# mattmireles/Mamba-ASR

Hardware: AMD Instinct MI355X
Metric: encoder audio-frames/sec (ConMamba-large, L=4000) (higher is better)
Workload: dtype bf16; 1 GPU; conmamba_large_ctc: encoder forward, 64 utterances x 4000 frames (1000 scan steps) per GPU, random-init weights; global_batch=64, frames_per_utterance=4000, parallelism=utterance shards x1 (no collective in forward), launch=hipGraph replay, streams=2 (join)

## Files before the change

### mamba_asr_amd/csrc/cnn_front.hip

```cpp
#include "cm_common.h"

namespace {

typedef __attribute__((ext_vector_type(8))) __bf16 bf16x8;
typedef __attribute__((ext_vector_type(2))) __bf16 bf16x2;
typedef __attribute__((ext_vector_type(4))) float f32x4;
typedef __attribute__((ext_vector_type(2))) float f32x2;

constexpr int F0 = 80;
constexpr int C1 = 64, F1 = 40, F1P = 42;
constexpr int C2 = 32, F2 = 20;
constexpr int TT = 4;
constexpr int NR = 2 * TT + 1;
constexpr int CS = 68;
constexpr int OTS = 36;
constexpr int FW = 84;
constexpr int NB = (TT * F2 + 15) / 16;

__device__ __forceinline__ int reflect_idx(int i, int n) { return i < 0 ? -i : (i >= n ? 2 * n - 2 - i : i); }
__device__ __forceinline__ float wave_sum64(float v) {
    v = cm_group_sum<16>(v);
    v += __shfl_xor(v, 16, 64);
    v += __shfl_xor(v, 32, 64);
    return v;
}
__device__ __forceinline__ uint32_t pack2(float a, float b) {
    return __builtin_bit_cast(uint32_t, __builtin_convertvector(f32x2{a, b}, bf16x2));
}

struct front_lds {
    uint16_t rows[NR][F1P][CS];
    float ot[NB * 16][OTS];
    float fin[8][3][2][FW];
    float ln1[2][F1 * C1];
    bf16x8 wfrag[2][18][64];
};

__global__ __launch_bounds__(512) void cnn_front_kernel(const cm_cnn_front_args p, int T1, int T2, int tiles_per_utt, int chunk, int chunks_per_utt,
                                                        int nchunks) {
    extern __shared__ __attribute__((aligned(16))) unsigned char smem[];
    front_lds &L = *reinterpret_cast<front_lds *>(smem);
    const int tid = threadIdx.x, lane = tid & 63;
    const int wave = __builtin_amdgcn_readfirstlane(tid >> 6);
    const int l15 = lane & 15, lq = lane >> 4;
    const int T = p.T, T1P = T1 + 2;

    const uint16_t *W2 = reinterpret_cast<const uint16_t *>(p.w2);
    for (int i = tid; i < 2 * 18 * 64; i += 512) {
        const int cb = i / (18 * 64), ks = (i / 64) % 18, ln = i % 64;
        L.wfrag[cb][ks][ln] = *reinterpret_cast<const bf16x8 *>(W2 + ((int64_t)(cb * 16 + (ln & 15)) * 9 + (ks >> 1)) * C1 + (ks & 1) * 32 + (ln >> 4) * 8);
    }
    float4 bias2[2];
#pragma unroll
    for (int cb = 0; cb < 2; ++cb)
        bias2[cb] = p.b2 ? *reinterpret_cast<const float4 *>(p.b2 + cb * 16 + lq * 4) : make_float4(0.f, 0.f, 0.f, 0.f);
    const int cp = lane & 31, fh = lane >> 5;
    f32x2 w1[9];
#pragma unroll
    for (int k = 0; k < 9; ++k) w1[k] = f32x2{p.w1[(2 * cp) * 9 + k], p.w1[(2 * cp + 1) * 9 + k]};
    const float b1a = p.b1 ? p.b1[2 * cp] : 0.f, b1b = p.b1 ? p.b1[2 * cp + 1] : 0.f;
    for (int i = tid; i < F1 * C1; i += 512) { L.ln1[0][i] = p.ln1_g[i]; L.ln1[1][i] = p.ln1_b[i]; }

    const int pidx = min(wave * 16 + l15, TT * F2 - 1);
    const int pr = pidx / F2, pf = pidx % F2;
    uint16_t *out = reinterpret_cast<uint16_t *>(p.out);

    auto fetch_rows = [&](const float *feats, int tp, float (&r)[4]) {
        const int t1 = reflect_idx(min(tp, T1P - 1) - 1, T1);
#pragma unroll
        for (int k = 0; k < 4; ++k) {
            const int idx = lane + 64 * k;
            r[k] = 0.f;
            if (idx < 3 * 82) {
                const int rr = idx / 82, fc = idx - rr * 82;
                r[k] = feats[(int64_t)reflect_idx(2 * t1 + rr - 1, T) * F0 + reflect_idx(fc - 1, F0)];
            }
        }
    };
    auto stage_rows = [&](const float (&r)[4]) {
#pragma unroll
        for (int k = 0; k < 4; ++k) {
            const int idx = lane + 64 * k;
            if (idx < 3 * 82) {
                const int rr = idx / 82, fc = idx % 82;
                L.fin[wave][rr][0][fc] = r[k];
                if (fc >= 2) L.fin[wave][rr][1][fc - 2] = r[k];
            }
        }
    };
    auto block1_row = [&](int slot) {
        float v[2 * (F1 / 2)];
        float s = 0.f;
#pragma unroll
        for (int i = 0; i < F1 / 2; ++i) {
            f32x2 a2 = {b1a, b1b};
#pragma unroll
            for (int dt = 0; dt < 3; ++dt) {
                const f32x4 xv = *reinterpret_cast<const f32x4 *>(&L.fin[wave][dt][fh][4 * i]);
#pragma unroll
                for (int df = 0; df < 3; ++df) a2 = __builtin_elementwise_fma(w1[dt * 3 + df], f32x2{xv[df], xv[df]}, a2);
            }
            v[2 * i] = a2.x; v[2 * i + 1] = a2.y;
            s += a2.x + a2.y;
            if (i & 1) __builtin_amdgcn_sched_barrier(0);
        }
        const float mean = wave_sum64(s) * (1.f / (F1 * C1));
        float sq = 0.f;
#pragma unroll
        for (int i = 0; i < F1; ++i) { v[i] -= mean; sq = fmaf(v[i], v[i], sq); }
        const float rstd = rsqrtf(wave_sum64(sq) * (1.f / (F1 * C1)) + p.eps1);
#pragma unroll
        for (int i = 0; i < F1 / 2; ++i) {
            const int f1 = 2 * i + fh, o = f1 * C1 + 2 * cp;
            const float2 g = *reinterpret_cast<const float2 *>(&L.ln1[0][o]);
            const float2 bt = *reinterpret_cast<const float2 *>(&L.ln1[1][o]);
            float y0 = fmaf(v[2 * i] * rstd, g.x, bt.x), y1 = fmaf(v[2 * i + 1] * rstd, g.y, bt.y);
            y0 = y0 > 0.f ? y0 : p.slope * y0;
            y1 = y1 > 0.f ? y1 : p.slope * y1;
            const uint32_t pk = pack2(y0, y1);
            *reinterpret_cast<uint32_t *>(&L.rows[slot][f1 + 1][2 * cp]) = pk;
            if (f1 == 1) *reinterpret_cast<uint32_t *>(&L.rows[slot][0][2 * cp]) = pk;
            if (f1 == F1 - 2) *reinterpret_cast<uint32_t *>(&L.rows[slot][F1P - 1][2 * cp]) = pk;
        }
    };

    for (int ch = blockIdx.x; ch < nchunks; ch += gridDim.x) {
        const int b = ch / chunks_per_utt, tile0 = (ch % chunks_per_utt) * chunk;
        const int tile1 = min(tile0 + chunk, tiles_per_utt);
        const float *feats = p.feats + (int64_t)b * T * F0;
        float pre[4];
        __syncthreads();
        if (wave == 0) {
            fetch_rows(feats, 2 * TT * tile0, pre);
            stage_rows(pre);
            block1_row((2 * TT * tile0) % NR);
        }
        fetch_rows(feats, 2 * TT * tile0 + 1 + wave, pre);
        for (int tile = tile0; tile < tile1; ++tile) {
            const int tp0 = 2 * TT * tile, r0 = TT * tile;
            stage_rows(pre);
            if (tile + 1 < tile1) fetch_rows(feats, tp0 + 2 * TT + 1 + wave, pre);
            block1_row((tp0 + 1 + wave) % NR);
            cm_lds_barrier();
            if (wave < NB) {
                f32x4 acc0 = {0.f, 0.f, 0.f, 0.f}, acc1 = {0.f, 0.f, 0.f, 0.f};
                const uint16_t *fr[3];
#pragma unroll
                for (int dt = 0; dt < 3; ++dt) fr[dt] = &L.rows[(tp0 + 2 * pr + dt) % NR][2 * pf][lq * 8];
#pragma unroll
                for (int ks = 0; ks < 18; ++ks) {
                    const int tap = ks >> 1, dt = tap / 3, df = tap % 3;
                    const bf16x8 bfr = *reinterpret_cast<const bf16x8 *>(fr[dt] + df * CS + (ks & 1) * 32);
                    acc0 = __builtin_amdgcn_mfma_f32_16x16x32_bf16(L.wfrag[0][ks][lane], bfr, acc0, 0, 0, 0);
                    acc1 = __builtin_amdgcn_mfma_f32_16x16x32_bf16(L.wfrag[1][ks][lane], bfr, acc1, 0, 0, 0);
                }
                float *o = &L.ot[wave * 16 + l15][lq * 4];
                *reinterpret_cast<float4 *>(o) = make_float4(acc0[0] + bias2[0].x, acc0[1] + bias2[0].y, acc0[2] + bias2[0].z, acc0[3] + bias2[0].w);
                *reinterpret_cast<float4 *>(o + 16) = make_float4(acc1[0] + bias2[1].x, acc1[1] + bias2[1].y, acc1[2] + bias2[1].z, acc1[3] + bias2[1].w);
            }
            cm_lds_barrier();
            if (wave < TT && r0 + wave < T2) {
                constexpr int nfeat = F2 * C2;
                const float *orow = &L.ot[wave * F2][0];
                float2 vv[nfeat / 128];
                float s = 0.f;
#pragma unroll
                for (int k = 0; k < nfeat / 128; ++k) {
                    const int i = lane + 64 * k;
                    vv[k] = *reinterpret_cast<const float2 *>(orow + (i >> 4) * OTS + 2 * (i & 15));
                    s += vv[k].x + vv[k].y;
                }
                const float mean = wave_sum64(s) * (1.f / nfeat);
                float sq = 0.f;
#pragma unroll
                for (int k = 0; k < nfeat / 128; ++k) {
                    vv[k].x -= mean; vv[k].y -= mean;
                    sq = fmaf(vv[k].x, vv[k].x, fmaf(vv[k].y, vv[k].y, sq));
                }
                const float rstd = rsqrtf(wave_sum64(sq) * (1.f / nfeat) + p.eps2);
                uint16_t *dst = out + ((int64_t)b * T2 + r0 + wave) * nfeat;
#pragma unroll
                for (int k = 0; k < nfeat / 128; ++k) {
                    const int i = lane + 64 * k;
                    const float2 g = *reinterpret_cast<const float2 *>(p.ln2_g + 2 * i);
                    const float2 bt = *reinterpret_cast<const float2 *>(p.ln2_b + 2 * i);
                    float y0 = fmaf(vv[k].x * rstd, g.x, bt.x), y1 = fmaf(vv[k].y * rstd, g.y, bt.y);
                    y0 = y0 > 0.f ? y0 : y0 * p.slope;
                    y1 = y1 > 0.f ? y1 : y1 * p.slope;
                    *reinterpret_cast<uint32_t *>(dst + 2 * i) = pack2(y0, y1);
                }
            }
            cm_lds_barrier();
        }
    }
}

}

extern "C" int cm_cnn_front(const cm_cnn_front_args *args) {
    CM_REQUIRE(args != nullptr, CM_EINVAL, "cnn_front: args is NULL");
    const cm_cnn_front_args &a = *args;
    CM_REQUIRE(a.batch > 0 && a.T >= 5 && a.feats && a.w1 && a.ln1_g && a.ln1_b && a.w2 && a.ln2_g && a.ln2_b && a.out, CM_EINVAL,
               "cnn_front: bad sizes or NULL tensor");
    CM_REQUIRE(a.F == F0 && a.C1 == C1 && a.C2 == C2, CM_EUNSUPPORTED, "cnn_front: only 80 bins, channels (64, 32) (got F %d, C %d, %d)", a.F,
               a.C1, a.C2);
    CM_REQUIRE(cm_aligned(a.w2, 16) && cm_aligned(a.out, 4) && cm_aligned(a.ln1_g, 8) && cm_aligned(a.ln1_b, 8) && cm_aligned(a.ln2_g, 8) &&
                   cm_aligned(a.ln2_b, 8) && (!a.b2 || cm_aligned(a.b2, 16)),
               CM_EALIGN, "cnn_front: w2 / b2 must be 16-byte aligned, LayerNorm parameters 8-byte aligned");
    const int T1 = (a.T + 1) / 2, T2 = (T1 + 2 - 3) / 2 + 1;
    const int tiles_per_utt = (T2 + TT - 1) / TT;
    const int chunk = 16;
    const int chunks_per_utt = (tiles_per_utt + chunk - 1) / chunk;
    const int64_t nchunks = (int64_t)a.batch * chunks_per_utt;
    CM_REQUIRE(nchunks <= 2147483647, CM_EINVAL, "cnn_front: too many chunks");
    static bool attr_done = false;
    if (!attr_done) {
        hipError_t e = hipFuncSetAttribute(reinterpret_cast<const void *>(cnn_front_kernel), hipFuncAttributeMaxDynamicSharedMemorySize, 150 * 1024);
        if (e != hipSuccess) {
            cm_set_error("cnn_front: hipFuncSetAttribute failed: %s", hipGetErrorString(e));
            return (int)e;
        }
        attr_done = true;
    }
    const int64_t grid = nchunks < 256 ? nchunks : 256;
    hipLaunchKernelGGL(cnn_front_kernel, dim3((unsigned)grid), dim3(512), sizeof(front_lds), reinterpret_cast<hipStream_t>(a.stream), a, T1, T2,
                       tiles_per_utt, chunk, chunks_per_utt, (int)nchunks);
    return cm_launch_status("cm_cnn_front");
}
```

### mamba_asr_amd/fused.py

```python
from __future__ import annotations

import os
from typing import Dict, Optional

import torch
import torch.nn.functional as F

from . import ops, weight_cache


class _LayerCache:

    def __init__(self, layer, dtype):
        self.dtype = dtype
        c = lambda t: t.detach().to(dtype).contiguous()
        f = lambda t: None if t is None else t.detach().float().contiguous()
        ffn = lambda m: dict(ln=(f(m[0].weight), f(m[0].bias), m[0].eps), w1=c(m[1].ffn[0].weight), b1=c(m[1].ffn[0].bias),
                             w2=c(m[1].ffn[3].weight), b2=c(m[1].ffn[3].bias), b1f=f(m[1].ffn[0].bias),
                             b2f=f(m[1].ffn[3].bias))
        self.ffn1, self.ffn2 = ffn(layer.ffn_module1), ffn(layer.ffn_module2)
        if ops.ffn_supported(self.ffn1["w1"].shape[1], self.ffn1["w1"].shape[0], dtype) and self.ffn1["w1"].is_cuda:
            for q in (self.ffn1, self.ffn2):
                q["w1p"], q["w2p"] = ops.PackedWeight(q["w1"], ops.FFN_LAYOUT), ops.PackedWeight(q["w2"], ops.FFN_LAYOUT)
                if ops.SMALL_FFN_ROWS > 0:
# ... 125 lines not shown
        xz = h @ c.in_proj.t()
        if c.in_bias is not None:
            xz = xz + c.in_bias
    xz3 = xz.view(batch, seqlen, 2 * E)
    ucat = torch.empty((batch, seqlen, 2 * E), dtype=xz.dtype, device=xz.device)
    xdbl = None
    if USE_CONV_XPROJ and USE_SCAN_ROWS and c.rows_mode and c.wx_packed is not None and xz.dtype == torch.bfloat16:
        xdbl = ops.conv_xproj(xz3[:, :, :E], c.dirs[0]["conv_w"], c.dirs[0]["conv_b"], c.dirs[1]["conv_w"], c.dirs[1]["conv_b"],
                              c.wx_packed[0], c.wx_packed[1], out_f=ucat[:, :, :E], out_b=ucat[:, :, E:])
    else:
        ops.conv_cl_fwd(xz3[:, :, :E], c.dirs[0]["conv_w"], c.dirs[0]["conv_b"], c.dirs[1]["conv_w"], c.dirs[1]["conv_b"],
                        True, out_f=ucat[:, :, :E], out_b=ucat[:, :, E:])
    ycat = torch.empty_like(ucat)
    dirs = _scan_dirs(c, ucat, ycat, batch, seqlen, xdbl)
    ops.scan_cl_fwd(dirs, z=xz3[:, :, E:], delta_softplus=True)
    y = ycat.view(rows, 2 * E) @ c.out_cat.t()
    if c.out_bias is not None:
        y = y + c.out_bias
    if c.gamma is not None:
        y = y * c.gamma.to(y.dtype)
    return y


USE_FUSED_FFN = os.environ.get("CM_FUSED_FFN", "1") == "1"


USE_LN_PW_GLU = os.environ.get("CM_LN_PW_GLU", "1") == "1"


def _layer_forward_ffn_fused(c, x, batch, seqlen, dtype, final_ln=None):
    D = x.shape[-1]
    f1, f2 = c.ffn1, c.ffn2
    if 0 < x.shape[0] <= ops.SMALL_FFN_ROWS and "w1s" in f1:
        f1 = dict(f1, w1p=f1["w1s"], w2p=f1["w2s"])
        f2 = dict(f2, w1p=f2["w1s"], w2p=f2["w2s"])
        inp = getattr(c, "in_packed_s", None)
    else:
        inp = c.in_packed
    if c.in_packed is not None:
        _, xz = ops.ffn_fused(x, f1["ln"], f1["w1p"], f1["b1f"], f1["w2p"], f1["b2f"], alpha=0.5, norm2=c.norm1, proj_w=inp)
        y = bimamba_fused(c, None, batch, seqlen, xz=xz)
    else:
        _, h = ops.ffn_fused(x, f1["ln"], f1["w1p"], f1["b1f"], f1["w2p"], f1["b2f"], alpha=0.5, norm2=c.norm1)
        y = bimamba_fused(c, h, batch, seqlen)
    if USE_LN_PW_GLU and c.pw_packed is not None and y.dtype == torch.bfloat16 and y.is_contiguous():
        gl = ops.ln_pw_glu(x, y, 1.0, c.cm_ln, c.pw_packed, c.pw_bf)
        g = ops.glu_dwconv_ln_gelu(gl.view(batch, seqlen, D), c.dw_w, c.dw_b, c.cm_ln2[0], c.cm_ln2[1], c.cm_ln2[2],
                                   weight_t=c.dw_wt, glu_done=True, lin_w=c.lin_packed, lin_b=c.lin_bf)
    else:
        _, h = ops.add_layernorm(x, y, 1.0, x_out=x, norm2=c.cm_ln, out_dtype=dtype)
        pw = torch.addmm(c.pw_b, h, c.pw_w.t()).view(batch, seqlen, 2 * D)
        g = ops.glu_dwconv_ln_gelu(pw, c.dw_w, c.dw_b, c.cm_ln2[0], c.cm_ln2[1], c.cm_ln2[2], weight_t=c.dw_wt,
                                   lin_w=c.lin_packed, lin_b=c.lin_bf)
    y = g if c.lin_packed is not None else torch.addmm(c.lin_b, g.view(-1, D), c.lin_w.t())
    if final_ln is not None:
        _, out = ops.ffn_fused(x, f2["ln"], f2["w1p"], f2["b1f"], f2["w2p"], f2["b2f"], alpha=0.5, addend=y.view(-1, D),
                               norm1=c.norm2, norm2=final_ln, h_dtype=torch.float32)
        return out, None
    ops.ffn_fused(x, f2["ln"], f2["w1p"], f2["b1f"], f2["w2p"], f2["b2f"], alpha=0.5, addend=y.view(-1, D), norm1=c.norm2,
                  want_h=False)
    return x, None


def layer_forward(layer, x, batch, seqlen, dtype, next_ln=None, final_ln=None):
    c = _cache(layer, dtype)
    D = x.shape[-1]
    if USE_FUSED_FFN and ops.ffn_supported(D, c.ffn1["w1"].shape[0], dtype) and c.ffn2["w1"].shape[0] == c.ffn1["w1"].shape[0]:
        return _layer_forward_ffn_fused(c, x, batch, seqlen, dtype, final_ln)
    _, h = ops.add_layernorm(x, None, norm2=c.ffn1["ln"], out_dtype=dtype)
    y = _ffn(x, h, c.ffn1, dtype)
    _, h = ops.add_layernorm(x, y, 0.5, x_out=x, norm2=c.norm1, out_dtype=dtype)
    y = bimamba_fused(c, h, batch, seqlen)
    _, h = ops.add_layernorm(x, y, 1.0, x_out=x, norm2=c.cm_ln, out_dtype=dtype)
    pw = torch.addmm(c.pw_b, h, c.pw_w.t()).view(batch, seqlen, 2 * D)
    g = ops.glu_dwconv_ln_gelu(pw, c.dw_w, c.dw_b, c.cm_ln2[0], c.cm_ln2[1], c.cm_ln2[2], weight_t=c.dw_wt)
    y = torch.addmm(c.lin_b, g.view(-1, D), c.lin_w.t())
    _, h = ops.add_layernorm(x, y, 1.0, x_out=x, norm2=c.ffn2["ln"], out_dtype=dtype)
    y = _ffn(x, h, c.ffn2, dtype)
    n1 = c.norm2
    if final_ln is not None:
        ops.add_layernorm(x, y, 0.5, x_out=x, norm1=n1, want_out=False)
        _, out = ops.add_layernorm(x, None, norm2=final_ln, out_dtype=torch.float32)
        return out, None
    ops.add_layernorm(x, y, 0.5, x_out=x, norm1=n1, want_out=False)
    return x, None



USE_NATIVE_GEMM = os.environ.get("CM_NATIVE_GEMM", "0") == "1"


def _native_gemms_ok(c: _LayerCache, D: int, dtype) -> bool:
    F_ = c.ffn1["w1"].shape[0]
    return (USE_NATIVE_GEMM and dtype == torch.bfloat16 and D == 256 and F_ % 256 == 0 and F_ % 64 == 0 and (2 * c.d_inner) % 256 == 0
            and c.gamma is None)


def layer_forward_native(layer, x, h, batch, seqlen, next_ln):
    c = _cache(layer, torch.bfloat16)
    D, E, R, N = x.shape[-1], c.d_inner, c.dt_rank, c.d_state
    rows = batch * seqlen
    g = ops.gemm_bf16
    u1 = g(h, c.ffn1["w1"], c.ffn1["b1f"], epilogue=1)
    h = g(u1, c.ffn1["w2"], c.ffn1["b2f"], epilogue=2, x=x, alpha=0.5, norm2=c.norm1)
    xz = g(h, c.in_proj, c.in_bias_f, epilogue=0)
    xz3 = xz.view(batch, seqlen, 2 * E)
    ucat = torch.empty((batch, seqlen, 2 * E), dtype=xz.dtype, device=xz.device)
    ops.conv_cl_fwd(xz3[:, :, :E], c.dirs[0]["conv_w"], c.dirs[0]["conv_b"], c.dirs[1]["conv_w"], c.dirs[1]["conv_b"],
                    True, out_f=ucat[:, :, :E], out_b=ucat[:, :, E:])
    ycat = torch.empty_like(ucat)
    dirs = _scan_dirs(c, ucat, ycat, batch, seqlen)
    ops.scan_cl_fwd(dirs, z=xz3[:, :, E:], delta_softplus=True)
    h = g(ycat.view(rows, 2 * E), c.out_cat, c.out_bias_f, epilogue=2, x=x, alpha=1.0, norm2=c.cm_ln)
    pw = g(h, c.pw_w, c.pw_bf, epilogue=0).view(batch, seqlen, 2 * D)
    gl = ops.glu_dwconv_ln_gelu(pw, c.dw_w, c.dw_b, c.cm_ln2[0], c.cm_ln2[1], c.cm_ln2[2], weight_t=c.dw_wt)
    h = g(gl.view(rows, D), c.lin_w, c.lin_bf, epilogue=2, x=x, alpha=1.0, norm2=c.ffn2["ln"])
    u2 = g(h, c.ffn2["w1"], c.ffn2["b1f"], epilogue=1)
    return g(u2, c.ffn2["w2"], c.ffn2["b2f"], epilogue=2, x=x, alpha=0.5, norm1=c.norm2, norm2=next_ln,
             want_out=next_ln is not None)


N_STREAMS = int(os.environ.get("CM_STREAMS", "2"))
STREAM_MODE = os.environ.get("CM_STREAM_MODE", "join")
_side_streams = {}


def _encoder_forward_joined(encoder, src, dtype, ns, paired=False):
    batch, seqlen, D = src.shape
    if dtype != torch.bfloat16 or not USE_FUSED_FFN or not (USE_CONV_XPROJ and USE_SCAN_ROWS and USE_LN_PW_GLU):
        return None
    caches = [_cache(layer, dtype) for layer in encoder.layers]
    for c in caches:
        if not (ops.ffn_supported(D, c.ffn1["w1"].shape[0], dtype) and c.ffn2["w1"].shape[0] == c.ffn1["w1"].shape[0] and c.rows_mode
                and c.wx_packed is not None and c.pw_packed is not None and c.in_bias is None and c.out_bias is None and c.gamma is None):
            return None
    dev = src.device
    cur = torch.cuda.current_stream(dev)
    pool = _side_streams.setdefault(dev.index, [])
    while len(pool) < ns - 1:
        pool.append(torch.cuda.Stream(device=dev))
    streams = [cur] + pool[:ns - 1]
    edges = [int(round(i * batch / ns)) for i in range(ns + 1)]
    parts = [(edges[i], edges[i + 1]) for i in range(ns) if edges[i + 1] > edges[i]]
    E = caches[0].d_inner
    n = len(encoder.layers)
    fin = (encoder.norm.norm.weight.detach().float(), encoder.norm.norm.bias.detach().float(), encoder.norm.norm.eps)
    with torch.autocast("cuda", enabled=False):
        x = src.detach().float().reshape(batch * seqlen, D).contiguous()
        if x.data_ptr() == src.data_ptr():
            x = x.clone()
        xz = torch.empty((batch, seqlen, 2 * E), dtype=dtype, device=dev)
        ucat, ycat = torch.empty_like(xz), torch.empty_like(xz)
        xdbl = torch.empty((batch, seqlen, 96), dtype=dtype, device=dev)
        outs = [None] * len(parts)

        def fork():
            for st in streams[1:len(parts)]:
                st.wait_stream(cur)

        def join():
            for st in streams[1:len(parts)]:
                cur.wait_stream(st)

        fork()
        gate = None
        for li, c in enumerate(caches):
            f1, f2 = c.ffn1, c.ffn2
            for pi, (b0, b1) in enumerate(parts):
                with torch.cuda.stream(streams[pi]):
                    xp = x[b0 * seqlen:b1 * seqlen]
                    if c.in_packed is not None:
                        ops.ffn_fused(xp, f1["ln"], f1["w1p"], f1["b1f"], f1["w2p"], f1["b2f"], alpha=0.5, norm2=c.norm1,
                                      proj_w=c.in_packed, proj_out=xz[b0:b1].view(-1, 2 * E))
                    else:
                        _, h = ops.ffn_fused(xp, f1["ln"], f1["w1p"], f1["b1f"], f1["w2p"], f1["b2f"], alpha=0.5, norm2=c.norm1)
                        torch.mm(h, c.in_proj.t(), out=xz[b0:b1].view(-1, 2 * E))
                    ops.conv_xproj(xz[b0:b1, :, :E], c.dirs[0]["conv_w"], c.dirs[0]["conv_b"], c.dirs[1]["conv_w"], c.dirs[1]["conv_b"],
                                   c.wx_packed[0], c.wx_packed[1], out_f=ucat[b0:b1, :, :E], out_b=ucat[b0:b1, :, E:], xdbl=xdbl[b0:b1])
            if paired:
                for pi, (b0, b1) in enumerate(parts):
                    with torch.cuda.stream(streams[pi]):
                        if gate is not None:
                            streams[pi].wait_event(gate)
                        ops.scan_cl_fwd(_scan_dirs(c, ucat[b0:b1], ycat[b0:b1], b1 - b0, seqlen, xdbl[b0:b1]), z=xz[b0:b1, :, E:],
                                        delta_softplus=True)
                        gate = torch.cuda.Event()
                        gate.record(streams[pi])
            else:
                join()
                ops.scan_cl_fwd(_scan_dirs(c, ucat, ycat, batch, seqlen, xdbl), z=xz[:, :, E:], delta_softplus=True)
                fork()
            for pi, (b0, b1) in enumerate(parts):
                with torch.cuda.stream(streams[pi]):
                    xp = x[b0 * seqlen:b1 * seqlen]
                    y = ycat[b0:b1].view(-1, 2 * E) @ c.out_cat.t()
                    gl = ops.ln_pw_glu(xp, y, 1.0, c.cm_ln, c.pw_packed, c.pw_bf)
                    g = ops.glu_dwconv_ln_gelu(gl.view(b1 - b0, seqlen, D), c.dw_w, c.dw_b, c.cm_ln2[0], c.cm_ln2[1], c.cm_ln2[2],
                                               weight_t=c.dw_wt, glu_done=True, lin_w=c.lin_packed, lin_b=c.lin_bf)
                    yl = g.view(-1, D) if c.lin_packed is not None else torch.addmm(c.lin_b, g.view(-1, D), c.lin_w.t())
                    if li == n - 1:
                        _, outs[pi] = ops.ffn_fused(xp, f2["ln"], f2["w1p"], f2["b1f"], f2["w2p"], f2["b2f"], alpha=0.5, addend=yl,
                                                    norm1=c.norm2, norm2=fin, h_dtype=torch.float32)
                    else:
                        ops.ffn_fused(xp, f2["ln"], f2["w1p"], f2["b1f"], f2["w2p"], f2["b2f"], alpha=0.5, addend=yl, norm1=c.norm2,
                                      want_h=False)
        join()
        for o in outs[1:]:
            o.record_stream(cur)
        return torch.cat(outs, dim=0).view(batch, seqlen, D)


@torch.no_grad()
def encoder_forward(encoder, src, dtype: Optional[torch.dtype] = None, streams: Optional[int] = None):
    if dtype is None:
        dtype = torch.get_autocast_dtype("cuda") if torch.is_autocast_enabled("cuda") else torch.float32
    ns = min(N_STREAMS, max(1, src.shape[0] // 16)) if streams is None else streams
    if ns > 1 and src.shape[0] >= 2 * 8 and STREAM_MODE in ("join", "pair"):
        out = _encoder_forward_joined(encoder, src, dtype, ns, paired=STREAM_MODE == "pair")
        if out is not None:
            return out
    if ns > 1 and src.shape[0] >= 2 * 8:
        dev = src.device
        cur = torch.cuda.current_stream(dev)
        pool = _side_streams.setdefault(dev.index, [torch.cuda.Stream(device=dev) for _ in range(ns - 1)])
        chunks = list(torch.chunk(src, ns, dim=0))
        outs = [None] * len(chunks)
        for i in range(1, len(chunks)):
            pool[i - 1].wait_stream(cur)
            with torch.cuda.stream(pool[i - 1]):
                outs[i] = encoder_forward(encoder, chunks[i], dtype, streams=1)
        outs[0] = encoder_forward(encoder, chunks[0], dtype, streams=1)
        for i in range(1, len(chunks)):
            cur.wait_stream(pool[i - 1])
            outs[i].record_stream(cur)
        return torch.cat(outs, dim=0)
    batch, seqlen, D = src.shape
    with torch.autocast("cuda", enabled=False):
        x = src.detach().float().reshape(batch * seqlen, D).contiguous()
        if x.data_ptr() == src.data_ptr():
            x = x.clone()
        n = len(encoder.layers)
        fin = (encoder.norm.norm.weight.detach().float(), encoder.norm.norm.bias.detach().float(), encoder.norm.norm.eps)
        caches = [_cache(layer, dtype) for layer in encoder.layers]
        if all(_native_gemms_ok(c, D, dtype) for c in caches):
            _, h = ops.add_layernorm(x, None, norm2=caches[0].ffn1["ln"], out_dtype=dtype)
            for i, layer in enumerate(encoder.layers):
                h = layer_forward_native(layer, x, h, batch, seqlen, caches[i + 1].ffn1["ln"] if i + 1 < n else None)
            _, out = ops.add_layernorm(x, None, norm2=fin, out_dtype=torch.float32)
            return out.view(batch, seqlen, D)
        out = x
        for i, layer in enumerate(encoder.layers):
            out, _ = layer_forward(layer, x, batch, seqlen, dtype, final_ln=fin if i == n - 1 else None)
        return out.view(batch, seqlen, D)


USE_CNN_FRONT = os.environ.get("CM_CNN_FRONT", "1") == "1"


def _frontend_bundle(model, dtype):
    b0, b1 = model.CNN.blocks
    lin = model.Transformer.custom_src_module.layers[0].w
    return dict(w2=b1.conv.weight.detach().to(dtype).contiguous(memory_format=torch.channels_last),
                b2=b1.conv.bias.detach().to(dtype), b2f=b1.conv.bias.detach().float().contiguous(),
                w2_ohwi=b1.conv.weight.detach().to(dtype).permute(0, 2, 3, 1).contiguous(),
                ln2=(b1.norm.norm.weight.detach().float().reshape(-1).contiguous(),
                     b1.norm.norm.bias.detach().float().reshape(-1).contiguous(), b1.norm.norm.eps),
                lin_w=lin.weight.detach().to(dtype).contiguous(), lin_b=lin.bias.detach().to(dtype))


_FRONTEND = weight_cache.Kind("_cm_frontend_cache", graphs_read=False, build=_frontend_bundle)


def _frontend_cache(model, dtype):
    return _FRONTEND.lookup(model, _params_key(dtype, model.CNN, model.Transformer.custom_src_module), dtype)


@torch.no_grad()
def asr_encode(model, wavs, wav_lens, dtype: Optional[torch.dtype] = None):
    if dtype is None:
        dtype = torch.get_autocast_dtype("cuda") if torch.is_autocast_enabled("cuda") else torch.float32
    with torch.autocast("cuda", enabled=False):
        feats = model.compute_features(wavs, norm=(model.normalize.glob_mean, model.normalize.glob_std))
        c = _frontend_cache(model, dtype)
        b0 = model.CNN.blocks[0]
        if (USE_CNN_FRONT and dtype == torch.bfloat16 and ops.cnn_front_supported(feats, b0.conv.weight, c["w2_ohwi"])
                and b0.norm.norm.weight.numel() == 40 * 64):
            src = ops.cnn_front(feats, b0.conv.weight, b0.conv.bias, b0.norm.norm.weight, b0.norm.norm.bias, b0.norm.norm.eps,
                                c["w2_ohwi"], c["b2f"], c["ln2"][0], c["ln2"][1], c["ln2"][2], 0.01)
            batch, t2 = src.shape[0], src.shape[1]
            x = torch.addmm(c["lin_b"], src.view(batch * t2, -1), c["lin_w"].t())
            return encoder_forward(model.Transformer.encoder, x.view(batch, t2, -1), dtype)
        y1 = ops.cnn_block1(feats, b0.conv.weight, b0.conv.bias, b0.norm.norm.weight, b0.norm.norm.bias,
                            b0.norm.norm.eps, 0.01, out_dtype=dtype, pad_out=1)
        if dtype == torch.bfloat16 and tuple(c["w2_ohwi"].shape) == (32, 3, 3, 64):
            src = ops.cnn_block2(y1, c["w2_ohwi"], c["b2f"], c["ln2"][0], c["ln2"][1], c["ln2"][2], 0.01)
            batch, t2 = src.shape[0], src.shape[1]
            x = torch.addmm(c["lin_b"], src.view(batch * t2, -1), c["lin_w"].t())
            return encoder_forward(model.Transformer.encoder, x.view(batch, t2, -1), dtype)
        y2 = F.conv2d(y1.permute(0, 3, 1, 2), c["w2"], c["b2"], stride=2)
        y2 = y2.permute(0, 2, 3, 1)
        if not y2.is_contiguous():
            y2 = y2.contiguous()
        batch, t2 = y2.shape[0], y2.shape[1]
        _, src = ops.add_layernorm(None, y2.reshape(batch * t2, -1), norm2=c["ln2"], out_dtype=dtype, out_act=1)
        x = torch.addmm(c["lin_b"], src, c["lin_w"].t())
        return encoder_forward(model.Transformer.encoder, x.view(batch, t2, -1), dtype)


class GraphedEncode:

    def __init__(self, model, wavs, wav_lens, dtype=torch.bfloat16, warmup: int = 2):
        self.model, self.dtype = model, dtype
        self.wavs, self.lens = wavs.clone(), wav_lens.clone()
        side = torch.cuda.Stream(device=wavs.device)
        side.wait_stream(torch.cuda.current_stream(wavs.device))
        with torch.cuda.stream(side):
            for _ in range(warmup):
                self._run()
        torch.cuda.current_stream(wavs.device).wait_stream(side)
        self.graph = torch.cuda.CUDAGraph()
        with torch.cuda.graph(self.graph):
            self.out = self._run()

    def _run(self):
        with torch.no_grad(), torch.autocast("cuda", dtype=self.dtype, enabled=self.dtype != torch.float32):
            return self.model.encode(self.wavs, self.lens)

    def __call__(self, wavs=None, wav_lens=None):
        if wavs is not None:
            self.wavs.copy_(wavs)
        if wav_lens is not None:
            self.lens.copy_(wav_lens)
        self.graph.replay()
        return self.out
```

### mamba_asr_amd/ops.py

```python
from __future__ import annotations

import ctypes as ct
from typing import Optional, Tuple

import math
import os

import torch

from . import _native as N
from . import weight_cache
from .weight_cache import invalidate_caches

_DT = {torch.float32: N.CM_F32, torch.bfloat16: N.CM_BF16, torch.float16: N.CM_F16}


DETERMINISTIC = os.environ.get("CM_DETERMINISTIC", "1") == "1"


LAUNCH_LOG: Optional[list] = None


def _launch(name: str, fn, args, units: int = 0):
    log = LAUNCH_LOG
# ... 1362 lines not shown
    b, l, d2 = inp.shape
    d = d2 if glu_done else d2 // 2
    w = _f32c(weight).reshape(d, -1)
    bs, g, bt = _f32c(bias), _f32c(ln_weight), _f32c(ln_bias)
    out = torch.empty((b, l, d), dtype=inp.dtype, device=inp.device)
    a = N.GluDwconvArgs()
    a.batch, a.seqlen, a.dim, a.ksize, a.io_dtype, a.glu_done = b, l, d, w.shape[1], _DT[inp.dtype], int(bool(glu_done))
    a.in_, a.weight, a.bias, a.ln_g, a.ln_b, a.eps, a.out = _ptr(inp), _ptr(w), _ptr(bs), _ptr(g), _ptr(bt), float(eps), _ptr(out)
    wt = w.t().contiguous() if weight_t is None else weight_t
    if wt.dtype != torch.float32 or wt.shape != (w.shape[1], d) or not wt.is_contiguous():
        raise RuntimeError("glu_dwconv_ln_gelu: weight_t must be a contiguous fp32 (k, dim) tensor")
    a.weight_t = _ptr(wt)
    if lin_w is not None:
        if not isinstance(lin_w, PackedWeight) or lin_w.shape != (d, d) or lin_b is None:
            raise RuntimeError("glu_dwconv_ln_gelu: lin_w must be a PackedWeight of shape (dim, dim), with lin_b")
        lb = _f32c(lin_b)
        a.lin_w, a.lin_b = _ptr(lin_w.data), _ptr(lb)
    a.stream, a.variant = _stream(), int(variant)
    _launch("cm_glu_dwconv_ln_gelu", N.lib().cm_glu_dwconv_ln_gelu, a, units=b * l)
    return out


def cnn_block1(feats, weight, bias, ln_weight, ln_bias, eps=1e-5, slope=0.01, out_dtype=torch.bfloat16, pad_out=1):
    _dev_check(feats, weight, bias, ln_weight, ln_bias)
    feats = feats.float().contiguous()
    b, t, f = feats.shape
    w, bs, g, bt = _f32c(weight), _f32c(bias), _f32c(ln_weight), _f32c(ln_bias)
    cch = w.shape[0]
    t1, f1 = (t + 1) // 2, (f + 1) // 2
    out = torch.empty((b, t1 + 2 * pad_out, f1 + 2 * pad_out, cch), dtype=out_dtype, device=feats.device)
    a = N.CnnBlock1Args()
    a.batch, a.T, a.F, a.C, a.io_dtype, a.pad_out = b, t, f, cch, _DT[out_dtype], pad_out
    a.feats, a.weight, a.bias, a.ln_g, a.ln_b, a.eps, a.slope, a.out = (_ptr(feats), _ptr(w), _ptr(bs), _ptr(g), _ptr(bt),
                                                                          float(eps), float(slope), _ptr(out))
    a.stream = _stream()
    _launch("cm_cnn_block1", N.lib().cm_cnn_block1, a, units=b * t)
    return out


def cnn_front_supported(feats, w1, w2_ohwi) -> bool:
    return (feats.shape[-1] == 80 and tuple(w1.shape) == (64, 1, 3, 3) and tuple(w2_ohwi.shape) == (32, 3, 3, 64)
            and w2_ohwi.dtype == torch.bfloat16 and feats.shape[1] >= 5)


def cnn_front(feats, w1, b1, ln1_w, ln1_b, eps1, w2_ohwi, b2, ln2_w, ln2_b, eps2, slope=0.01):
    _dev_check(feats, w1, b1, ln1_w, ln1_b, w2_ohwi, b2, ln2_w, ln2_b)
    feats = feats.float().contiguous()
    if not cnn_front_supported(feats, w1, w2_ohwi) or not w2_ohwi.is_contiguous():
        raise RuntimeError("cnn_front: needs 80 bins, a (64, 1, 3, 3) first conv and a contiguous bf16 (32, 3, 3, 64) second conv")
    b, t, f = feats.shape
    t1 = (t + 1) // 2
    t2 = (t1 - 1) // 2 + 1
    w1f, b1f, g1, bt1 = _f32c(w1), _f32c(b1), _f32c(ln1_w).reshape(-1), _f32c(ln1_b).reshape(-1)
    b2f, g2, bt2 = _f32c(b2), _f32c(ln2_w).reshape(-1), _f32c(ln2_b).reshape(-1)
    if g1.numel() != 40 * 64 or g2.numel() != 20 * 32:
        raise RuntimeError("cnn_front: LayerNorm parameters must have 40*64 and 20*32 elements")
    out = torch.empty((b, t2, 640), dtype=torch.bfloat16, device=feats.device)
    a = N.CnnFrontArgs()
    a.batch, a.T, a.F, a.C1, a.C2 = b, t, f, 64, 32
    a.feats, a.w1, a.b1, a.ln1_g, a.ln1_b = _ptr(feats), _ptr(w1f), _ptr(b1f), _ptr(g1), _ptr(bt1)
    a.w2, a.b2, a.ln2_g, a.ln2_b = _ptr(w2_ohwi), _ptr(b2f), _ptr(g2), _ptr(bt2)
    a.eps1, a.eps2, a.slope, a.out, a.stream = float(eps1), float(eps2), float(slope), _ptr(out), _stream()
    _launch("cm_cnn_front", N.lib().cm_cnn_front, a, units=b * t)
    return out


def cnn_block2(y1, weight_ohwi, bias, ln_weight, ln_bias, eps=1e-5, slope=0.01):
    _dev_check(y1, weight_ohwi, bias, ln_weight, ln_bias)
    if y1.dtype != torch.bfloat16 or not y1.is_contiguous() or y1.dim() != 4:
        raise RuntimeError("cnn_block2: input must be a contiguous bf16 (batch, T, F, C) tensor")
    if weight_ohwi.dtype != torch.bfloat16 or not weight_ohwi.is_contiguous() or weight_ohwi.dim() != 4:
        raise RuntimeError("cnn_block2: weight must be a contiguous bf16 (C_out, 3, 3, C_in) tensor")
    b, t, f, cin = y1.shape
    cout = weight_ohwi.shape[0]
    if tuple(weight_ohwi.shape[1:]) != (3, 3, cin):
        raise RuntimeError("cnn_block2: weight shape does not match the input channels / 3x3 taps")
    t2, f2 = (t - 3) // 2 + 1, (f - 3) // 2 + 1
    bs, g, bt = _f32c(bias), _f32c(ln_weight).reshape(-1), _f32c(ln_bias).reshape(-1)
    if g.numel() != f2 * cout or bt.numel() != f2 * cout:
        raise RuntimeError("cnn_block2: LayerNorm parameters must have F2 * C_out elements")
    out = torch.empty((b, t2, f2 * cout), dtype=torch.bfloat16, device=y1.device)
    a = N.CnnBlock2Args()
    a.batch, a.T_in, a.F_in, a.C_in, a.C_out = b, t, f, cin, cout
    a.in_, a.weight, a.bias, a.ln_g, a.ln_b, a.eps, a.slope, a.out = (_ptr(y1), _ptr(weight_ohwi), _ptr(bs), _ptr(g), _ptr(bt),
                                                                      float(eps), float(slope), _ptr(out))
    a.stream = _stream()
    _launch("cm_cnn_block2", N.lib().cm_cnn_block2, a, units=b * t2)
    return out


def gemm_supported(m: int, n: int, k: int, epilogue: int) -> bool:
    return k % 64 == 0 and n % 256 == 0 and (epilogue != 2 or n == 256)


def gemm_bf16(a, w, bias=None, epilogue=0, x=None, alpha=1.0, norm1=None, norm2=None, want_out=True):
    _dev_check(a, w, bias, x)
    if a.dtype != torch.bfloat16 or w.dtype != torch.bfloat16 or a.dim() != 2 or a.stride(1) != 1 or not w.is_contiguous():
        raise RuntimeError("gemm_bf16: a must be a (M, K) bf16 row-major view and w a contiguous (N, K) bf16 tensor")
    m, k = a.shape
    n = w.shape[0]
    g = N.GemmArgs()
    g.M, g.N, g.K, g.epilogue = m, n, k, epilogue
    g.A, g.lda, g.W, g.ldw, g.bias = _ptr(a), a.stride(0), _ptr(w), w.stride(0), _ptr(bias)
    out = None
    if epilogue != 2 or want_out:
        out = torch.empty((m, n), dtype=torch.bfloat16, device=a.device)
        g.out, g.ldo = _ptr(out), n
    if epilogue == 2:
        if x is None or x.dtype != torch.float32 or not x.is_contiguous() or x.shape != (m, n):
            raise RuntimeError("gemm_bf16: epilogue 2 needs a contiguous fp32 residual x of shape (M, N)")
        g.x, g.alpha = _ptr(x), float(alpha)
        if norm1 is not None:
            g.g1, g.b1, g.eps1 = _ptr(norm1[0]), _ptr(norm1[1]), float(norm1[2])
        if norm2 is not None:
            g.g2, g.b2, g.eps2 = _ptr(norm2[0]), _ptr(norm2[1]), float(norm2[2])
    g.stream = _stream()
    _launch("cm_gemm_bf16", N.lib().cm_gemm_bf16, g, units=m)
    return out


def ffn_supported(d_model: int, hidden: int, dtype) -> bool:
    return dtype == torch.bfloat16 and d_model == 256 and hidden >= 256 and hidden % 256 == 0


FFN_LAYOUT = 32 if os.environ.get("CM_FFN_MFMA32", "0") == "1" else 16
SMALL_FFN_ROWS = int(os.environ.get("CM_FFN_SMALL_ROWS", "0"))


class PackedWeight:

    def __init__(self, w: torch.Tensor, layout: int = 16):
        _dev_check(w)
        if w.dtype != torch.bfloat16 or w.dim() != 2:
            raise RuntimeError("PackedWeight: expected a 2-D bf16 tensor")
        if layout not in (16, 32):
            raise RuntimeError("PackedWeight: layout must be 16 or 32")
        w = w.contiguous()
        self.shape = tuple(w.shape)
        self.layout = layout
        self.data = torch.empty(w.numel(), dtype=torch.bfloat16, device=w.device)
        self.repack_(w)

    def repack_(self, w: torch.Tensor) -> "PackedWeight":
        if w.dtype != torch.bfloat16 or tuple(w.shape) != self.shape or w.device != self.data.device:
            raise RuntimeError("PackedWeight.repack_: expected a bf16 tensor of the packed shape on the image's device")
        w = w.contiguous()
        fn = N.lib().cm_ffn_pack_weights if self.layout == 16 else N.lib().cm_ffn_pack_weights32
        rc = fn(_ptr(w), w.shape[0], w.shape[1], _ptr(self.data), _stream())
        N.check(rc, "cm_ffn_pack_weights")
        return self


def ffn_fused(x, pre_norm, w1, b1, w2, b2, alpha=0.5, addend=None, add_scale=1.0, norm1=None, norm2=None,
              x_out=None, want_h=True, h_dtype=torch.bfloat16, proj_w=None, proj_b=None, proj_out=None, train=None, tokens=None):
    _dev_check(x, b1, b2, addend, proj_b)
    rows, d = x.shape
    if x.dtype != torch.float32 or not x.is_contiguous():
        raise RuntimeError("ffn_fused: x must be a contiguous fp32 (rows, 256) tensor")
    if d != 256:
        raise RuntimeError(f"ffn_fused: d_model must be 256 (got {d})")
    lay = w1.layout if isinstance(w1, PackedWeight) else (w2.layout if isinstance(w2, PackedWeight) else (16 if train is not None else FFN_LAYOUT))
    w1 = w1 if isinstance(w1, PackedWeight) else PackedWeight(w1, lay)
    w2 = w2 if isinstance(w2, PackedWeight) else PackedWeight(w2, lay)
    if w1.shape[1] != d or w2.shape != (d, w1.shape[0]):
        raise RuntimeError("ffn_fused: weight shapes do not match x")
    if w1.layout != w2.layout or (proj_w is not None and isinstance(proj_w, PackedWeight) and proj_w.layout != w1.layout):
        raise RuntimeError("ffn_fused: w1, w2 and proj_w must be packed in the same layout")
    if train is not None and w1.layout != 16:
        raise RuntimeError("ffn_fused: the training forward takes layout-16 weights")
    for t in (b1, b2) + tuple(pre_norm[:2]):
        if t.dtype != torch.float32:
            raise RuntimeError("ffn_fused: biases and LayerNorm parameters must be fp32")
    a = N.FfnArgs()
    a.rows, a.dim, a.hidden = rows, d, w1.shape[0]
    a.x, a.pre_g, a.pre_b, a.pre_eps = _ptr(x), _ptr(pre_norm[0]), _ptr(pre_norm[1]), float(pre_norm[2])
    a.w1, a.b1, a.w2, a.b2, a.alpha = _ptr(w1.data), _ptr(b1), _ptr(w2.data), _ptr(b2), float(alpha)
    a.layout = 1 if w1.layout == 32 else 0
    if w1.layout == 32:
        a.tokens = int(tokens) if tokens else (32 if rows <= SMALL_FFN_ROWS else 64)
    if addend is not None:
        if addend.dtype != torch.bfloat16 or not addend.is_contiguous() or addend.shape != x.shape:
            raise RuntimeError("ffn_fused: addend must be a contiguous bf16 tensor shaped like x")
        a.addend, a.add_scale = _ptr(addend), float(add_scale)
    if norm1 is not None:
        a.n1_g, a.n1_b, a.n1_eps = _ptr(norm1[0]), _ptr(norm1[1]), float(norm1[2])
    if norm2 is not None:
        a.n2_g, a.n2_b, a.n2_eps = _ptr(norm2[0]), _ptr(norm2[1]), float(norm2[2])
    xo = x if x_out is None else x_out
    a.x_out = _ptr(xo)
    h = None
    if train is not None:
        if addend is not None or norm1 is not None or norm2 is not None or proj_w is not None:
            raise RuntimeError("ffn_fused: the training forward takes no addend / norm1 / norm2 / projection")
        pre = torch.empty((rows, w1.shape[0]), dtype=torch.bfloat16, device=x.device)
        xn = torch.empty((rows, d), dtype=torch.bfloat16, device=x.device)
        stats = torch.empty((2, rows), dtype=torch.float32, device=x.device)
        a.pre_out, a.xn_out, a.stats_out = _ptr(pre), _ptr(xn), _ptr(stats)
        a.p1, a.p2, a.seed1, a.seed2 = float(train[0]), float(train[1]), int(train[2]), int(train[3])
        a.seed_epoch = _seed_epoch_ptr()
        a.stream = _stream()
        _launch("cm_ffn_fused", N.lib().cm_ffn_fused, a, units=rows)
        return xo, (pre, xn, stats)
    if proj_w is not None:
        if not isinstance(proj_w, PackedWeight) or proj_w.shape[1] != d or proj_w.shape[0] % 256 or proj_w.shape[0] > 4096:
            raise RuntimeError("ffn_fused: proj_w must be a PackedWeight of shape (P, 256), P a multiple of 256 up to 4096")
        h = proj_out if proj_out is not None else torch.empty((rows, proj_w.shape[0]), dtype=torch.bfloat16, device=x.device)
        if h.shape != (rows, proj_w.shape[0]) or h.dtype != torch.bfloat16 or not h.is_contiguous():
            raise RuntimeError("ffn_fused: proj_out must be a contiguous bf16 (rows, P) tensor")
        _dev_check(h)
        pb = _f32c(proj_b)
        a.proj_w, a.proj_b, a.proj_out, a.proj_dim = _ptr(proj_w.data), _ptr(pb), _ptr(h), proj_w.shape[0]
    elif want_h:
        h = torch.empty((rows, d), dtype=h_dtype, device=x.device)
        a.h_out, a.h_dtype = _ptr(h), _DT[h_dtype]
    a.stream = _stream()
    _launch("cm_ffn_fused", N.lib().cm_ffn_fused, a, units=rows)
    return xo, h


_BANDS = {}


def _mel_bands(fb: torch.Tensor):
    key = (fb.data_ptr(), tuple(fb.shape))
    if key not in _BANDS:
        nz = (fb != 0)
        idx = torch.arange(fb.shape[0], device=fb.device)[:, None]
        lo = torch.where(nz, idx, fb.shape[0]).amin(0).to(torch.int32)
        hi = (torch.where(nz, idx, -1).amax(0) + 1).to(torch.int32)
        lo = torch.minimum(lo, hi)
        width = (hi - lo).to(torch.int64)
        off = torch.zeros(fb.shape[1] + 1, dtype=torch.int64, device=fb.device)
        off[1:] = torch.cumsum(width, 0)
        total = int(off[-1])
        packed = None
        if 0 < total <= 4096:
            m_of = torch.repeat_interleave(torch.arange(fb.shape[1], device=fb.device), width)
            f_of = torch.arange(total, device=fb.device) - off[m_of] + lo.to(torch.int64)[m_of]
            packed = fb[f_of, m_of].contiguous()
        _BANDS[key] = (lo.contiguous(), hi.contiguous(), off.to(torch.int32).contiguous(), packed)
    return _BANDS[key]


def fbank_from_stft(spec, fbank, amin=1e-10, top_db=80.0, mean=None, std=None):
    _dev_check(spec, fbank, mean, std)
    sr = torch.view_as_real(spec) if spec.is_complex() else spec
    if sr.dtype != torch.float32 or sr.stride(3) != 1 or any(st % 2 for st in sr.stride()[:3]):
        sr = sr.float().contiguous()
    b, nf, t, _ = sr.shape
    fb = _f32c(fbank)
    m = fb.shape[1]
    db = torch.empty((b, t, m), dtype=torch.float32, device=sr.device)
    umax = torch.empty((b,), dtype=torch.float32, device=sr.device)
    part = torch.empty((b, (t + 15) // 16), dtype=torch.float32, device=sr.device)
    a = N.FbankArgs()
    a.batch, a.n_freq, a.frames, a.n_mels = b, nf, t, m
    a.spec, a.fbank, a.db, a.umax, a.amin, a.top_db = _ptr(sr), _ptr(fb), _ptr(db), _ptr(umax), float(amin), float(top_db)
    mean, std = _f32c(mean), _f32c(std)
    a.mean, a.std = _ptr(mean), _ptr(std)
    lo, hi, off, packed = _mel_bands(fb)
    a.band_lo, a.band_hi = _ptr(lo), _ptr(hi)
    if packed is not None:
        a.band_off, a.band_w = _ptr(off), _ptr(packed)
    a.spec_bs, a.spec_fs, a.spec_ts = sr.stride(0) // 2, sr.stride(1) // 2, sr.stride(2) // 2
    a.umax_part = _ptr(part)
    a.stream = _stream()
    _launch("cm_fbank_mel_db", N.lib().cm_fbank_mel_db, a, units=b * t)
    _launch("cm_fbank_finish", N.lib().cm_fbank_finish, a, units=b * t)
    return db


_FFT_TABLES = {}


def _fft_tables(window: torch.Tensor, n_fft: int):
    key = (window.data_ptr(), window.numel(), n_fft, str(window.device))
    if key not in _FFT_TABLES:
        win = torch.zeros(n_fft, dtype=torch.float32, device=window.device)
        left = (n_fft - window.numel()) // 2
        win[left:left + window.numel()] = window.float()
        k = torch.arange(n_fft, dtype=torch.float64)
        ang = -2.0 * torch.pi * k / n_fft
        tw = torch.stack([torch.cos(ang), torch.sin(ang)], dim=1).to(torch.float32).to(window.device).contiguous()
        _FFT_TABLES[key] = (win, tw)
    return _FFT_TABLES[key]


def fbank_wav_supported(n_fft: int, hop: int, n_mels: int) -> bool:
    return n_fft == 512 and hop % 2 == 0 and n_mels <= 128


def fbank_from_wav(wav, window, n_fft, hop, fbank, amin=1e-10, top_db=80.0, mean=None, std=None):
    _dev_check(wav, window, fbank, mean, std)
    if wav.dtype != torch.float32 or wav.dim() != 2 or wav.stride(1) != 1:
        wav = wav.float().contiguous()
    if wav.stride(0) % 2:
        wav = wav.contiguous() if wav.shape[1] % 2 == 0 else torch.nn.functional.pad(wav, (0, 1))[:, :wav.shape[1]]
    b, ns = wav.shape
    fb = _f32c(fbank)
    nf, m = fb.shape
    t = 1 + ns // hop
    win, tw = _fft_tables(window, n_fft)
    lo, hi, off, packed = _mel_bands(fb)
    if packed is None:
        raise RuntimeError("fbank_from_wav: filterbank is not banded (no packed band weights)")
    db = torch.empty((b, t, m), dtype=torch.float32, device=wav.device)
    umax = torch.empty((b,), dtype=torch.float32, device=wav.device)
    part = torch.empty((b, (t + 15) // 16), dtype=torch.float32, device=wav.device)
    a = N.FbankArgs()
    a.batch, a.n_freq, a.frames, a.n_mels = b, nf, t, m
    a.fbank, a.db, a.umax, a.amin, a.top_db = _ptr(fb), _ptr(db), _ptr(umax), float(amin), float(top_db)
    mean, std = _f32c(mean), _f32c(std)
    a.mean, a.std = _ptr(mean), _ptr(std)
    a.band_lo, a.band_hi, a.band_off, a.band_w = _ptr(lo), _ptr(hi), _ptr(off), _ptr(packed)
    a.umax_part = _ptr(part)
    a.wav, a.window, a.twiddle, a.wav_bs = _ptr(wav), _ptr(win), _ptr(tw), wav.stride(0)
    a.samples, a.hop, a.n_fft = ns, hop, n_fft
    a.stream = _stream()
    _launch("cm_fbank_wav", N.lib().cm_fbank_wav, a, units=b * t)
    _launch("cm_fbank_finish", N.lib().cm_fbank_finish, a, units=b * t)
    return db


def spec_drop_(feats, start, length, dim, fill):
    _dev_check(feats, start, length, fill)
    if feats.dtype != torch.float32 or not feats.is_contiguous():
        raise RuntimeError("spec_drop_: feats must be contiguous fp32")
    start, length = start.to(torch.int32).contiguous(), length.to(torch.int32).contiguous()
    fill = fill.reshape(1).float()
    b, t, m = feats.shape
    a = N.SpecDropArgs()
    a.batch, a.frames, a.n_mels, a.n_masks, a.dim = b, t, m, start.shape[1], dim
    a.feats, a.start, a.length, a.fill = _ptr(feats), _ptr(start), _ptr(length), _ptr(fill)
    a.stream = _stream()
    _launch("cm_spec_drop", N.lib().cm_spec_drop, a, units=b * t)
    return feats
```

Before: 19.58 million audio-frames/s.

## Overlap CNN front LayerNorm with next tile's MFMA and write encoder output in place

```diff
diff --git a/mamba_asr_amd/csrc/cnn_front.hip b/mamba_asr_amd/csrc/cnn_front.hip
--- a/mamba_asr_amd/csrc/cnn_front.hip
+++ b/mamba_asr_amd/csrc/cnn_front.hip
@@ -16,6 +16,7 @@
 constexpr int OTS = 36;
 constexpr int FW = 84;
 constexpr int NB = (TT * F2 + 15) / 16;
+static_assert(NB < 8 && 2 * (8 - NB) >= TT, "the waves the MFMA phase leaves idle take at most two LayerNorm rows each");
 
 __device__ __forceinline__ int reflect_idx(int i, int n) { return i < 0 ? -i : (i >= n ? 2 * n - 2 - i : i); }
 __device__ __forceinline__ float wave_sum64(float v) {
@@ -30,7 +31,7 @@
 
 struct front_lds {
     uint16_t rows[NR][F1P][CS];
-    float ot[NB * 16][OTS];
+    float ot[2][NB * 16][OTS];
     float fin[8][3][2][FW];
     float ln1[2][F1 * C1];
     bf16x8 wfrag[2][18][64];
@@ -124,6 +125,49 @@
         }
     };
 
+    float2 g2[F2 * C2 / 128], bt2[F2 * C2 / 128];
+#pragma unroll
+    for (int k = 0; k < F2 * C2 / 128; ++k) {
+        g2[k] = *reinterpret_cast<const float2 *>(p.ln2_g + 2 * (lane + 64 * k));
+        bt2[k] = *reinterpret_cast<const float2 *>(p.ln2_b + 2 * (lane + 64 * k));
+    }
+    auto block2_ln = [&](int buf, int st, int64_t orow) {
+        constexpr int nfeat = F2 * C2;
+        const float *src = &L.ot[buf][st * F2][0];
+        float2 vv[nfeat / 128];
+        float s = 0.f;
+#pragma unroll
+        for (int k = 0; k < nfeat / 128; ++k) {
+            const int i = lane + 64 * k;
+            vv[k] = *reinterpret_cast<const float2 *>(src + (i >> 4) * OTS + 2 * (i & 15));
+            s += vv[k].x + vv[k].y;
+        }
+        const float mean = wave_sum64(s) * (1.f / nfeat);
+        float sq = 0.f;
+#pragma unroll
+        for (int k = 0; k < nfeat / 128; ++k) {
+            vv[k].x -= mean; vv[k].y -= mean;
+            sq = fmaf(vv[k].x, vv[k].x, fmaf(vv[k].y, vv[k].y, sq));
+        }
+        const float rstd = rsqrtf(wave_sum64(sq) * (1.f / nfeat) + p.eps2);
+        uint16_t *dst = out + orow * nfeat;
+#pragma unroll
+        for (int k = 0; k < nfeat / 128; ++k) {
+            const int i = lane + 64 * k;
+            float y0 = fmaf(vv[k].x * rstd, g2[k].x, bt2[k].x), y1 = fmaf(vv[k].y * rstd, g2[k].y, bt2[k].y);
+            y0 = y0 > 0.f ? y0 : y0 * p.slope;
+            y1 = y1 > 0.f ? y1 : y1 * p.slope;
+            *reinterpret_cast<uint32_t *>(dst + 2 * i) = pack2(y0, y1);
+        }
+    };
+    int q = 0, ln_cnt = 0;
+    int64_t ln_row = 0;
+    auto pending_ln = [&]() {
+        if (wave >= NB) {
+            for (int st = 2 * (wave - NB); st < min(2 * (wave - NB) + 2, ln_cnt); ++st) block2_ln((q - 1) & 1, st, ln_row + st);
+        }
+    };
+
     for (int ch = blockIdx.x; ch < nchunks; ch += gridDim.x) {
         const int b = ch / chunks_per_utt, tile0 = (ch % chunks_per_utt) * chunk;
         const int tile1 = min(tile0 + chunk, tiles_per_utt);
@@ -154,45 +198,18 @@
                     acc0 = __builtin_amdgcn_mfma_f32_16x16x32_bf16(L.wfrag[0][ks][lane], bfr, acc0, 0, 0, 0);
                     acc1 = __builtin_amdgcn_mfma_f32_16x16x32_bf16(L.wfrag[1][ks][lane], bfr, acc1, 0, 0, 0);
                 }
-                float *o = &L.ot[wave * 16 + l15][lq * 4];
+                float *o = &L.ot[q & 1][wave * 16 + l15][lq * 4];
                 *reinterpret_cast<float4 *>(o) = make_float4(acc0[0] + bias2[0].x, acc0[1] + bias2[0].y, acc0[2] + bias2[0].z, acc0[3] + bias2[0].w);
                 *reinterpret_cast<float4 *>(o + 16) = make_float4(acc1[0] + bias2[1].x, acc1[1] + bias2[1].y, acc1[2] + bias2[1].z, acc1[3] + bias2[1].w);
             }
+            pending_ln();
+            ln_row = (int64_t)b * T2 + r0;
+            ln_cnt = min(TT, T2 - r0);
+            ++q;
             cm_lds_barrier();
-            if (wave < TT && r0 + wave < T2) {
-                constexpr int nfeat = F2 * C2;
-                const float *orow = &L.ot[wave * F2][0];
-                float2 vv[nfeat / 128];
-                float s = 0.f;
-#pragma unroll
-                for (int k = 0; k < nfeat / 128; ++k) {
-                    const int i = lane + 64 * k;
-                    vv[k] = *reinterpret_cast<const float2 *>(orow + (i >> 4) * OTS + 2 * (i & 15));
-                    s += vv[k].x + vv[k].y;
-                }
-                const float mean = wave_sum64(s) * (1.f / nfeat);
-                float sq = 0.f;
-#pragma unroll
-                for (int k = 0; k < nfeat / 128; ++k) {
-                    vv[k].x -= mean; vv[k].y -= mean;
-                    sq = fmaf(vv[k].x, vv[k].x, fmaf(vv[k].y, vv[k].y, sq));
-                }
-                const float rstd = rsqrtf(wave_sum64(sq) * (1.f / nfeat) + p.eps2);
-                uint16_t *dst = out + ((int64_t)b * T2 + r0 + wave) * nfeat;
-#pragma unroll
-                for (int k = 0; k < nfeat / 128; ++k) {
-                    const int i = lane + 64 * k;
-                    const float2 g = *reinterpret_cast<const float2 *>(p.ln2_g + 2 * i);
-                    const float2 bt = *reinterpret_cast<const float2 *>(p.ln2_b + 2 * i);
-                    float y0 = fmaf(vv[k].x * rstd, g.x, bt.x), y1 = fmaf(vv[k].y * rstd, g.y, bt.y);
-                    y0 = y0 > 0.f ? y0 : y0 * p.slope;
-                    y1 = y1 > 0.f ? y1 : y1 * p.slope;
-                    *reinterpret_cast<uint32_t *>(dst + 2 * i) = pack2(y0, y1);
-                }
-            }
-            cm_lds_barrier();
-        }
-    }
+        }
+    }
+    pending_ln();
 }
 
 }
diff --git a/mamba_asr_amd/fused.py b/mamba_asr_amd/fused.py
--- a/mamba_asr_amd/fused.py
+++ b/mamba_asr_amd/fused.py
@@ -301,7 +301,7 @@
         xz = torch.empty((batch, seqlen, 2 * E), dtype=dtype, device=dev)
         ucat, ycat = torch.empty_like(xz), torch.empty_like(xz)
         xdbl = torch.empty((batch, seqlen, 96), dtype=dtype, device=dev)
-        outs = [None] * len(parts)
+        out = torch.empty((batch * seqlen, D), dtype=torch.float32, device=dev)
 
         def fork():
             for st in streams[1:len(parts)]:
@@ -348,15 +348,13 @@
                                                weight_t=c.dw_wt, glu_done=True, lin_w=c.lin_packed, lin_b=c.lin_bf)
                     yl = g.view(-1, D) if c.lin_packed is not None else torch.addmm(c.lin_b, g.view(-1, D), c.lin_w.t())
                     if li == n - 1:
-                        _, outs[pi] = ops.ffn_fused(xp, f2["ln"], f2["w1p"], f2["b1f"], f2["w2p"], f2["b2f"], alpha=0.5, addend=yl,
-                                                    norm1=c.norm2, norm2=fin, h_dtype=torch.float32)
+                        ops.ffn_fused(xp, f2["ln"], f2["w1p"], f2["b1f"], f2["w2p"], f2["b2f"], alpha=0.5, addend=yl, norm1=c.norm2,
+                                      norm2=fin, h_dtype=torch.float32, h_out=out[b0 * seqlen:b1 * seqlen])
                     else:
                         ops.ffn_fused(xp, f2["ln"], f2["w1p"], f2["b1f"], f2["w2p"], f2["b2f"], alpha=0.5, addend=yl, norm1=c.norm2,
                                       want_h=False)
         join()
-        for o in outs[1:]:
-            o.record_stream(cur)
-        return torch.cat(outs, dim=0).view(batch, seqlen, D)
+        return out.view(batch, seqlen, D)
 
 
 @torch.no_grad()
diff --git a/mamba_asr_amd/ops.py b/mamba_asr_amd/ops.py
--- a/mamba_asr_amd/ops.py
+++ b/mamba_asr_amd/ops.py
@@ -1538,7 +1538,8 @@
 
 
 def ffn_fused(x, pre_norm, w1, b1, w2, b2, alpha=0.5, addend=None, add_scale=1.0, norm1=None, norm2=None,
-              x_out=None, want_h=True, h_dtype=torch.bfloat16, proj_w=None, proj_b=None, proj_out=None, train=None, tokens=None):
+              x_out=None, want_h=True, h_dtype=torch.bfloat16, proj_w=None, proj_b=None, proj_out=None, train=None, tokens=None,
+              h_out=None):
     _dev_check(x, b1, b2, addend, proj_b)
     rows, d = x.shape
     if x.dtype != torch.float32 or not x.is_contiguous():
@@ -1597,7 +1598,10 @@
         pb = _f32c(proj_b)
         a.proj_w, a.proj_b, a.proj_out, a.proj_dim = _ptr(proj_w.data), _ptr(pb), _ptr(h), proj_w.shape[0]
     elif want_h:
-        h = torch.empty((rows, d), dtype=h_dtype, device=x.device)
+        h = h_out if h_out is not None else torch.empty((rows, d), dtype=h_dtype, device=x.device)
+        if h.shape != (rows, d) or h.dtype != h_dtype or not h.is_contiguous():
+            raise RuntimeError("ffn_fused: h_out must be a contiguous (rows, 256) tensor of h_dtype")
+        _dev_check(h)
         a.h_out, a.h_dtype = _ptr(h), _DT[h_dtype]
     a.stream = _stream()
     _launch("cm_ffn_fused", N.lib().cm_ffn_fused, a, units=rows)
```

Result: no change. 19.67 million audio-frames/s, median of 6 (+0.4%).
